# irvingzhang0512/tf_eager_object_detection

Measured on AMD Instinct MI355X. Metric: images/sec, higher is better.
Workload: dtype f32

## Files before the change

tf_eager_object_detection_amd/csrc/nms.hip:

```cpp
#include <stddef.h>
#include <string.h>

#include <algorithm>
#include <mutex>

#include "conv_diag.h"

#define NMS_CHUNK 4096
#define NMS_SEL_MAX (2 * NMS_CHUNK)
#define NMS_WORDS (NMS_CHUNK / 64)
#define SEL_BINS 4096
#define SEL_REPL 8
#define SEL_BLOCK 256
#define SEL_ITEMS 8
#define SEL_TILE (SEL_BLOCK * SEL_ITEMS)
#define PREP_ITEMS 2
#define PREP_TILE (256 * PREP_ITEMS)

typedef unsigned long long u64;

#define SCAN_LDS_BLOCKS 24
#define SCAN_LDS_CAND (SCAN_LDS_BLOCKS * 64)
#define SCAN_LDS_WORDS (SCAN_LDS_BLOCKS * (SCAN_LDS_BLOCKS - 1) / 2 * 64)
#define SCAN_LDS_SLACK_WORDS (8 * 64)
#define SCAN_DYN_LDS ((SCAN_LDS_WORDS + SCAN_LDS_SLACK_WORDS) * 8)
#define SCAN_MAT_OFF(cb, nblk) (64 * ((cb) * ((nblk)-1) - (cb) * ((cb)-1) / 2))

struct NmsState {
  int32_t n_invalid;
  int32_t kept;
  int32_t pos;
  int32_t done;
  int32_t chunk_m;
  int32_t sel_count;
  int32_t reserved0;
  int32_t sel_b1;
  uint32_t sel_below1;
  int32_t sel_b2;
  int32_t sel_overflow;
  uint32_t sel_below;
  int32_t pad[4];
};

#define SEL_COARSE 64
struct NmsHeader {
  NmsState st;
  int32_t n_invalid_acc;
  int32_t pad_acc[15];
  uint32_t hist0[SEL_REPL][SEL_COARSE];
  uint32_t hist1[SEL_REPL][SEL_BINS];
  uint32_t hist2[SEL_BINS];
  uint32_t hist3[256];
};

enum { PREP_NMS = 0, PREP_RP = 1, PREP_FPN = 2, PREP_FRCNN = 3 };

struct PrepParams {
  int n;
  PerImg<const float4*> boxes_in;
  PerImg<const float*> deltas;
  PerImg<const float*> scores;
  PerImg<const float2*> logits;
  Vec4 means, stds;
  float wmax, hmax;
  PerImg<float4*> boxes_out;
  PerImg<uint32_t*> keys;
  PerImg<NmsHeader*> hdr;
  FpnAnchorParams fpn;
};

__global__ void __launch_bounds__(256) k_zero_headers(PerImg<NmsHeader*> hdr_) {
  uint4* d = reinterpret_cast<uint4*>(hdr_.v[blockIdx.y]);
  const int i = blockIdx.x * 256 + threadIdx.x;
  if (i < (int)(sizeof(NmsHeader) / 16)) d[i] = make_uint4(0, 0, 0, 0);
}

template <int MODE>
__device__ __forceinline__ float4 d_prep_box(const PrepParams& p, int img, int e) {
  if (MODE == PREP_NMS) return p.boxes_in.v[img][e];
  float4 a;
  if (MODE == PREP_FPN) {
    a = d_fpn_anchor(p.fpn, e);
  } else if (MODE == PREP_FRCNN) {
    const int ai = e % p.fpn.A, cell = e / p.fpn.A;
    const int x = cell % p.fpn.fw[0], y = cell / p.fpn.fw[0];
    const float sx = (float)(x * p.fpn.stride[0]), sy = (float)(y * p.fpn.stride[0]);
    a = make_float4(p.fpn.wh[ai * 4 + 0] + sx, p.fpn.wh[ai * 4 + 1] + sy, p.fpn.wh[ai * 4 + 2] + sx,
                    p.fpn.wh[ai * 4 + 3] + sy);
  } else {
    a = p.boxes_in.v[img][e];
  }
  const float4 d = reinterpret_cast<const float4*>(p.deltas.v[img])[e];
  const float d0 = d.x * p.stds.v[0] + p.means.v[0];
  const float d1 = d.y * p.stds.v[1] + p.means.v[1];
  const float d2 = d.z * p.stds.v[2] + p.means.v[2];
  const float d3 = d.w * p.stds.v[3] + p.means.v[3];
  float4 b = d_decode_box(a, d0, d1, d2, d3);
  return d_clip_box(b, 0.0f, p.wmax, p.hmax);
}

__device__ __forceinline__ float4 d_candidate_box(const PrepParams& p, int mode, int img, int e) {
  switch (mode) {
    case PREP_NMS: return d_prep_box<PREP_NMS>(p, img, e);
    case PREP_RP: return d_prep_box<PREP_RP>(p, img, e);
    case PREP_FRCNN: return d_prep_box<PREP_FRCNN>(p, img, e);
    default: return d_prep_box<PREP_FPN>(p, img, e);
  }
}

struct PrepItems {
  float sc[PREP_ITEMS];
  float2 lg[PREP_ITEMS];
};

template <int MODE>
__device__ __forceinline__ void d_prep_load(const PrepParams& p, const float* __restrict__ in_scores,
                                            const float2* __restrict__ in_logits, int tile, PrepItems* v) {
#pragma unroll
  for (int it = 0; it < PREP_ITEMS; ++it) {
    const int e = tile * PREP_TILE + it * 256 + threadIdx.x;
    const int ee = e < p.n ? e : 0;
    if (MODE == PREP_FPN) {
      v->lg[it] = in_logits[ee];
    } else if (MODE == PREP_FRCNN) {
      const int loc = ee / p.fpn.A, a = ee - loc * p.fpn.A;
      const float* row = reinterpret_cast<const float*>(in_logits) + (size_t)loc * 2 * p.fpn.A;
      v->lg[it] = make_float2(row[a], row[p.fpn.A + a]);
    } else {
      v->sc[it] = in_scores[ee];
    }
  }
}

__device__ __forceinline__ uint32_t d_row16_sum(uint32_t v) {
  v += (uint32_t)__builtin_amdgcn_update_dpp(0, (int)v, 0xB1, 0xF, 0xF, false);
  v += (uint32_t)__builtin_amdgcn_update_dpp(0, (int)v, 0x4E, 0xF, 0xF, false);
  v += (uint32_t)__builtin_amdgcn_update_dpp(0, (int)v, 0x141, 0xF, 0xF, false);
  v += (uint32_t)__builtin_amdgcn_update_dpp(0, (int)v, 0x140, 0xF, 0xF, false);
  return v;
}

template <int MODE, int T>
__global__ void __launch_bounds__(256) k_rp_prepare(PrepParams p) {
  const int img = blockIdx.y;
  const float* __restrict__ in_scores = p.scores.v[img];
  const float2* __restrict__ in_logits = p.logits.v[img];
  uint32_t* __restrict__ out_keys = p.keys.v[img];
  NmsHeader* hdr = p.hdr.v[img];
  __shared__ __attribute__((aligned(16))) uint32_t h[SEL_BINS];
  uint4* h4 = reinterpret_cast<uint4*>(h);
#pragma unroll
  for (int q = 0; q < SEL_BINS / 4 / 256; ++q) h4[q * 256 + threadIdx.x] = make_uint4(0, 0, 0, 0);
  PrepItems cur;
  d_prep_load<MODE>(p, in_scores, in_logits, blockIdx.x * T, &cur);
  __syncthreads();
  int invalid = 0;
#pragma unroll
  for (int t = 0; t < T; ++t) {
    const int tile = blockIdx.x * T + t;
    PrepItems nxt;
    if (t + 1 < T) d_prep_load<MODE>(p, in_scores, in_logits, tile + 1, &nxt);
#pragma unroll
    for (int it = 0; it < PREP_ITEMS; ++it) {
      const int e = tile * PREP_TILE + it * 256 + threadIdx.x;
      if (e < p.n) {
        float s;
        if (MODE == PREP_FPN || MODE == PREP_FRCNN) s = d_fg_prob(cur.lg[it].x, cur.lg[it].y);
        else s = cur.sc[it];
        const bool valid = s > -3.402823466e+38f;
        const uint32_t k = valid ? ~d_float_asc_key(s) : 0xFFFFFFFFu;
        out_keys[e] = k;
        invalid += valid ? 0 : 1;
        atomicAdd(&h[k >> 20], 1u);
      }
    }
    if (t + 1 < T) cur = nxt;
  }
  __syncthreads();
  const int repl = blockIdx.x % SEL_REPL;
  const int lane = threadIdx.x & 63;
#pragma unroll
  for (int q = 0; q < SEL_BINS / 4 / 256; ++q) {
    const int k4 = q * 256 + threadIdx.x;
    const uint4 c = h4[k4];
    uint32_t s = c.x + c.y + c.z + c.w;
    if (__ballot(s != 0)) {
      const int first = (k4 - lane) * 4;
#pragma unroll
      for (int i = 0; i < 4; ++i) {
        const uint32_t v = h[first + i * 64 + lane];
        if (v) atomicAdd(&hdr->hist1[repl][first + i * 64 + lane], v);
      }
    }
    s = d_row16_sum(s);
    if ((threadIdx.x & 15) == 0 && s) atomicAdd(&hdr->hist0[repl][k4 >> 4], s);
  }
  if (invalid) atomicAdd(&hdr->n_invalid_acc, invalid);
}

template <int REPL>
__device__ __forceinline__ void sel_find(const uint32_t* __restrict__ hist, uint32_t target, uint32_t* result,
                                         int* lds17) {
  uint32_t v[16];
#pragma unroll
  for (int q = 0; q < 16; ++q) v[q] = 0;
#pragma unroll
  for (int r = 0; r < REPL; ++r) {
    const uint4* h4 = reinterpret_cast<const uint4*>(hist + (size_t)r * SEL_BINS) + threadIdx.x * 4;
#pragma unroll
    for (int q = 0; q < 4; ++q) {
      const uint4 t = h4[q];
      v[q * 4 + 0] += t.x; v[q * 4 + 1] += t.y; v[q * 4 + 2] += t.z; v[q * 4 + 3] += t.w;
    }
  }
  uint32_t s = 0;
#pragma unroll
  for (int q = 0; q < 16; ++q) s += v[q];
  int total;
  const uint32_t excl = (uint32_t)block_excl_scan((int)s, lds17, &total);
  if ((uint32_t)total < target) target = (uint32_t)total;
  if (threadIdx.x == 0 && total == 0) { result[0] = SEL_BINS - 1; result[1] = 0; result[2] = 0; }
  if (s > 0 && excl < target && target <= excl + s) {
    uint32_t run = excl;
#pragma unroll
    for (int q = 0; q < 16; ++q) {
      if (run < target && target <= run + v[q]) {
        result[0] = threadIdx.x * 16 + q; result[1] = run; result[2] = v[q];
      }
      run += v[q];
    }
  }
  __syncthreads();
}

__device__ __forceinline__ void sel_find1_coarse(const NmsHeader* hdr, uint32_t target, uint32_t* res) {
  if (threadIdx.x < 64) {
    const int t = threadIdx.x;
    int c = 0;
#pragma unroll
    for (int r = 0; r < SEL_REPL; ++r) c += (int)hdr->hist0[r][t];
    const int inc = wave_incl_scan(c);
    const int total = __shfl(inc, 63);
    if (total == 0) {
      if (t == 0) { res[0] = SEL_BINS - 1; res[1] = 0; }
    } else {
      const int tgt = (int)(target > (uint32_t)total ? (uint32_t)total : target);
      const u64 hitc = __ballot(c > 0 && inc - c < tgt && tgt <= inc);
      const int cb = __builtin_ctzll(hitc);
      const int below_c = __shfl(inc - c, cb);
      int v = 0;
#pragma unroll
      for (int r = 0; r < SEL_REPL; ++r) v += (int)hdr->hist1[r][cb * 64 + t];
      const int inc2 = wave_incl_scan(v);
      const u64 hitf = __ballot(v > 0 && below_c + inc2 - v < tgt && tgt <= below_c + inc2);
      const int fb = __builtin_ctzll(hitf);
      const int below_f = __shfl(inc2 - v, fb);
      if (t == 0) { res[0] = (uint32_t)(cb * 64 + fb); res[1] = (uint32_t)(below_c + below_f); }
    }
  }
  __syncthreads();
}

__global__ void __launch_bounds__(SEL_BLOCK) k_sel_hist2(PerImg<NmsHeader*> hdr_, PerImg<const uint32_t*> keys_, int n,
                                                         uint32_t target) {
  NmsHeader* hdr = hdr_.v[blockIdx.y];
  const uint32_t* __restrict__ keys = keys_.v[blockIdx.y];
  __shared__ uint32_t h[SEL_BINS];
  __shared__ uint32_t res[2];
  uint32_t key[SEL_ITEMS];
#pragma unroll
  for (int it = 0; it < SEL_ITEMS; ++it) {
    const int e = blockIdx.x * SEL_TILE + it * SEL_BLOCK + threadIdx.x;
    key[it] = (e < n) ? keys[e] : 0u;
  }
  sel_find1_coarse(hdr, target, res);
  const uint32_t b1 = res[0];
  if (blockIdx.x == 0 && threadIdx.x == 0) {
    NmsState z;
    memset(&z, 0, sizeof(z));
    z.n_invalid = hdr->n_invalid_acc;
    z.sel_b1 = (int32_t)b1; z.sel_below1 = res[1];
    hdr->st = z;
    hdr->n_invalid_acc = 0;
  }
  bool match = false;
#pragma unroll
  for (int it = 0; it < SEL_ITEMS; ++it) {
    const int e = blockIdx.x * SEL_TILE + it * SEL_BLOCK + threadIdx.x;
    match = match || (e < n && (key[it] >> 20) == b1);
  }
  if (!__syncthreads_or(match ? 1 : 0)) return;
  for (int k = threadIdx.x; k < SEL_BINS; k += SEL_BLOCK) h[k] = 0;
  __syncthreads();
#pragma unroll
  for (int it = 0; it < SEL_ITEMS; ++it) {
    const int e = blockIdx.x * SEL_TILE + it * SEL_BLOCK + threadIdx.x;
    if (e < n && (key[it] >> 20) == b1) atomicAdd(&h[(key[it] >> 8) & 0xFFFu], 1u);
  }
  __syncthreads();
  for (int k = threadIdx.x; k < SEL_BINS; k += SEL_BLOCK) {
    const uint32_t c = h[k];
    if (c) atomicAdd(&hdr->hist2[k], c);
  }
}

__global__ void __launch_bounds__(SEL_BLOCK) k_sel_compact(PerImg<NmsHeader*> hdr_, PerImg<const uint32_t*> keys_, int n,
                                                           uint32_t target, uint32_t limit, PerImg<u64*> cand_) {
  NmsHeader* hdr = hdr_.v[blockIdx.y];
  const uint32_t* __restrict__ keys = keys_.v[blockIdx.y];
  u64* __restrict__ cand = cand_.v[blockIdx.y];
  __shared__ uint32_t res[3];
  __shared__ int lds17[17];
  const uint32_t b1 = (uint32_t)hdr->st.sel_b1;
  const uint32_t below1 = hdr->st.sel_below1;
  {
    static_assert(offsetof(NmsHeader, hist1) == offsetof(NmsHeader, hist0) + sizeof(uint32_t) * SEL_REPL * SEL_COARSE, "layout");
    uint4* z = reinterpret_cast<uint4*>(&hdr->hist0[0][0]);
    for (int i = blockIdx.x * SEL_BLOCK + threadIdx.x; i < SEL_REPL * (SEL_COARSE + SEL_BINS) / 4; i += gridDim.x * SEL_BLOCK)
      z[i] = make_uint4(0, 0, 0, 0);
  }
  uint32_t total_n = (uint32_t)n;
  uint32_t t2 = (target > total_n ? total_n : target) - below1;
  sel_find<1>(hdr->hist2, t2, res, lds17);
  const uint32_t b2 = res[0];
  const bool incl = (below1 + res[1] + res[2]) <= limit;
  if (blockIdx.x == 0 && threadIdx.x == 0) {
    hdr->st.sel_b2 = (int32_t)b2;
    hdr->st.sel_overflow = incl ? 0 : 1;
    hdr->st.sel_below = below1 + res[1];
  }
  __shared__ u64 stage[SEL_TILE];
  __shared__ int s_cnt, s_base;
  if (threadIdx.x == 0) s_cnt = 0;
  uint32_t key[SEL_ITEMS];
#pragma unroll
  for (int it = 0; it < SEL_ITEMS; ++it) {
    const int e = blockIdx.x * SEL_TILE + it * SEL_BLOCK + threadIdx.x;
    key[it] = (e < n) ? keys[e] : 0xFFFFFFFFu;
  }
  __syncthreads();
  const int lane = threadIdx.x & 63;
  const u64 lt_mask = (lane == 0) ? 0ull : (~0ull >> (64 - lane));
#pragma unroll
  for (int it = 0; it < SEL_ITEMS; ++it) {
    const int e = blockIdx.x * SEL_TILE + it * SEL_BLOCK + threadIdx.x;
    const uint32_t k = key[it];
    const uint32_t p1 = k >> 20, p2 = (k >> 8) & 0xFFFu;
    const bool sel = (e < n) && (p1 < b1 || (p1 == b1 && (p2 < b2 || (incl && p2 == b2))));
    const u64 bal = __ballot(sel);
    if (bal) {
      int base = 0;
      if (lane == __builtin_ctzll(bal)) base = atomicAdd(&s_cnt, (int)__popcll(bal));
      base = __shfl(base, __builtin_ctzll(bal));
      if (sel) stage[base + (int)__popcll(bal & lt_mask)] = ((u64)k << 32) | (uint32_t)e;
    }
  }
  __syncthreads();
  const int c = s_cnt;
  if (c == 0) return;
  if (threadIdx.x == 0) s_base = atomicAdd(&hdr->st.sel_count, c);
  __syncthreads();
  const int gb = s_base;
  for (int i = threadIdx.x; i < c; i += SEL_BLOCK)
    if (gb + i < NMS_SEL_MAX) cand[gb + i] = stage[i];
}

__global__ void __launch_bounds__(SEL_BLOCK) k_sel_tie_hist(PerImg<NmsHeader*> hdr_, PerImg<const uint32_t*> keys_, int n,
                                                            PerImg<unsigned short*> bh_) {
  NmsHeader* hdr = hdr_.v[blockIdx.y];
  if (!hdr->st.sel_overflow) return;
  const uint32_t* __restrict__ keys = keys_.v[blockIdx.y];
  unsigned short* __restrict__ bh = bh_.v[blockIdx.y] + (size_t)blockIdx.x * 256;
  __shared__ uint32_t h[256];
  const uint32_t pref = ((uint32_t)hdr->st.sel_b1 << 12) | (uint32_t)hdr->st.sel_b2;
  h[threadIdx.x] = 0;
  __syncthreads();
#pragma unroll
  for (int it = 0; it < SEL_ITEMS; ++it) {
    const int e = blockIdx.x * SEL_TILE + it * SEL_BLOCK + threadIdx.x;
    if (e < n) {
      const uint32_t k = keys[e];
      if ((k >> 8) == pref) atomicAdd(&h[k & 0xFFu], 1u);
    }
  }
  __syncthreads();
  const uint32_t c = h[threadIdx.x];
  bh[threadIdx.x] = (unsigned short)c;
  if (c) atomicAdd(&hdr->hist3[threadIdx.x], c);
}

__global__ void __launch_bounds__(SEL_BLOCK) k_sel_tie_take(PerImg<NmsHeader*> hdr_, PerImg<const uint32_t*> keys_, int n,
                                                            uint32_t limit, PerImg<const unsigned short*> bh_,
                                                            PerImg<u64*> cand_) {
  NmsHeader* hdr = hdr_.v[blockIdx.y];
  if (!hdr->st.sel_overflow) return;
  const uint32_t below = hdr->st.sel_below;
  if (below >= limit) return;
  const uint32_t quota = limit - below;
  const uint32_t* __restrict__ keys = keys_.v[blockIdx.y];
  const unsigned short* __restrict__ bh = bh_.v[blockIdx.y];
  u64* __restrict__ cand = cand_.v[blockIdx.y];
  __shared__ int lds17[17];
  __shared__ uint32_t s_b3, s_q3, s_pre;
  __shared__ int s_wave[4];
  __shared__ u64 stage[SEL_TILE];
  __shared__ int s_cnt, s_base;
  const uint32_t pref = ((uint32_t)hdr->st.sel_b1 << 12) | (uint32_t)hdr->st.sel_b2;
  const uint32_t hv = hdr->hist3[threadIdx.x];
  int total;
  const uint32_t excl = (uint32_t)block_excl_scan((int)hv, lds17, &total);
  if (threadIdx.x == 0) { s_b3 = 256; s_q3 = 0; s_pre = 0; s_cnt = 0; }
  __syncthreads();
  if (hv > 0 && excl < quota && quota <= excl + hv) { s_b3 = threadIdx.x; s_q3 = quota - excl; }
  __syncthreads();
  const uint32_t b3 = s_b3, q3 = s_q3;
  if (b3 < 256) {
    uint32_t mine = 0;
    for (int b = threadIdx.x; b < (int)blockIdx.x; b += SEL_BLOCK) mine += bh[(size_t)b * 256 + b3];
    int tot2;
    block_excl_scan((int)mine, lds17, &tot2);
    if (threadIdx.x == 0) s_pre = (uint32_t)tot2;
  }
  __syncthreads();
  uint32_t run = s_pre;
  const int lane = threadIdx.x & 63, wv = threadIdx.x >> 6;
  const u64 lt_mask = (lane == 0) ? 0ull : (~0ull >> (64 - lane));
  for (int it = 0; it < SEL_ITEMS; ++it) {
    const int e = blockIdx.x * SEL_TILE + it * SEL_BLOCK + threadIdx.x;
    const uint32_t k = (e < n) ? keys[e] : 0xFFFFFFFFu;
    const bool inbin = (e < n) && (k >> 8) == pref;
    const uint32_t v = k & 0xFFu;
    const bool tie = inbin && v == b3;
    const u64 tb = __ballot(tie);
    if (lane == 0) s_wave[wv] = (int)__popcll(tb);
    __syncthreads();
    uint32_t before = run;
    for (int q = 0; q < wv; ++q) before += (uint32_t)s_wave[q];
    const uint32_t my_rank = before + (uint32_t)__popcll(tb & lt_mask);
    const uint32_t all4 = (uint32_t)(s_wave[0] + s_wave[1] + s_wave[2] + s_wave[3]);
    const bool sel = inbin && (v < b3 || (tie && my_rank < q3));
    const u64 bal = __ballot(sel);
    if (bal) {
      int base = 0;
      if (lane == __builtin_ctzll(bal)) base = atomicAdd(&s_cnt, (int)__popcll(bal));
      base = __shfl(base, __builtin_ctzll(bal));
      if (sel) stage[base + (int)__popcll(bal & lt_mask)] = ((u64)k << 32) | (uint32_t)e;
    }
    run += all4;
    __syncthreads();
  }
  const int c = s_cnt;
  if (c == 0) return;
  if (threadIdx.x == 0) s_base = atomicAdd(&hdr->st.sel_count, c);
  __syncthreads();
  const int gb = s_base;
  for (int i = threadIdx.x; i < c; i += SEL_BLOCK)
    if (gb + i < NMS_SEL_MAX) cand[gb + i] = stage[i];
}

#define RANK_THREADS 1024
__global__ void __launch_bounds__(RANK_THREADS) k_sel_rank(PerImg<NmsHeader*> hdr_, int n, int cap0, PerImg<const u64*> cand_,
                                                          PrepParams prep, int mode, PerImg<uint32_t*> sel_idx_,
                                                          PerImg<float4*> sboxes_, PerImg<float4*> sorig_) {
  NmsHeader* hdr = hdr_.v[blockIdx.y];
  const u64* __restrict__ cand = cand_.v[blockIdx.y];
  uint32_t* __restrict__ sel_idx = sel_idx_.v[blockIdx.y];
  float4* __restrict__ sboxes = sboxes_.v[blockIdx.y];
  float4* __restrict__ sorig = sorig_.v[blockIdx.y];
  __shared__ u64 all[NMS_CHUNK];
  __shared__ int part[16][64];
  NmsState* st = &hdr->st;
  const int cnt = min(st->sel_count, NMS_SEL_MAX);
  if (blockIdx.x == 0 && threadIdx.x == 0) st->chunk_m = min(min(cnt, cap0), n - st->n_invalid);
  if (blockIdx.x == 0) {
    uint4* z = reinterpret_cast<uint4*>(hdr->hist2);
    for (int i = threadIdx.x; i < SEL_BINS / 4; i += RANK_THREADS) z[i] = make_uint4(0, 0, 0, 0);
    if (threadIdx.x < 256) hdr->hist3[threadIdx.x] = 0;
  }
  if (blockIdx.x * 64 >= cnt) return;
  const int lane = threadIdx.x & 63, w = threadIdx.x >> 6;
  const int i = blockIdx.x * 64 + lane;
  const u64 mine = (i < cnt) ? cand[i] : ~0ull;
  float4 bx = make_float4(0.0f, 0.0f, 0.0f, 0.0f);
  if (w == 0 && i < cnt) bx = d_candidate_box(prep, mode, blockIdx.y, (int)(uint32_t)mine);
  int c = 0;
  for (int t0 = 0; t0 < cnt; t0 += NMS_CHUNK) {
    const int tc = min(NMS_CHUNK, cnt - t0);
    __syncthreads();
    for (int k = threadIdx.x; k < tc; k += RANK_THREADS) all[k] = cand[t0 + k];
    __syncthreads();
    const int per = (tc + 15) >> 4;
    const int lo = w * per, hi = min(tc, lo + per);
    for (int j = lo; j < hi; ++j) c += (all[j] < mine) ? 1 : 0;
  }
  part[w][lane] = c;
  __syncthreads();
  if (w == 0 && i < cnt) {
    int r = 0;
#pragma unroll
    for (int k = 0; k < 16; ++k) r += part[k][lane];
    const uint32_t idx = (uint32_t)mine;
    sel_idx[r] = idx;
    if (r < cap0) {
      sboxes[r] = d_norm_box(bx);
      sorig[r] = bx;
    }
  }
}

__global__ void __launch_bounds__(256) k_nms_gather(PerImg<NmsState*> st_, int n, int cap, int from_sel,
                                                    PrepParams prep, int mode, PerImg<const uint32_t*> sorted_idx_,
                                                    PerImg<float4*> sboxes_, PerImg<float4*> sorig_) {
  NmsState* st = st_.v[blockIdx.y];
  const uint32_t* __restrict__ sorted_idx = sorted_idx_.v[blockIdx.y];
  float4* __restrict__ sboxes = sboxes_.v[blockIdx.y];
  float4* __restrict__ sorig = sorig_.v[blockIdx.y];
  const int pos = st->pos, nv = n - st->n_invalid;
  const int lim = from_sel ? min(nv, min(st->sel_count, NMS_SEL_MAX)) : nv;
  const int m = st->done ? 0 : max(0, min(cap, lim - pos));
  const int i = blockIdx.x * 256 + threadIdx.x;
  if (i == 0) st->chunk_m = m;
  if (i < m) {
    const float4 bx = d_candidate_box(prep, mode, blockIdx.y, (int)sorted_idx[pos + i]);
    sboxes[i] = d_norm_box(bx);
    sorig[i] = bx;
  }
}

__global__ void __launch_bounds__(256) k_nms_cross(PerImg<const NmsState*> st_, PerImg<const float4*> sboxes_,
                                                   PerImg<const float4*> kept_boxes_, float thr,
                                                   PerImg<u64*> removed_init_) {
  const NmsState* st = st_.v[blockIdx.y];
  const float4* __restrict__ sboxes = sboxes_.v[blockIdx.y];
  const float4* __restrict__ kept_boxes = kept_boxes_.v[blockIdx.y];
  u64* __restrict__ removed_init = removed_init_.v[blockIdx.y];
  __shared__ float4 kb[256];
  __shared__ float ka[256];
  const int m = st->chunk_m, nk = st->kept;
  if (blockIdx.x * 256 >= m) return;
  const int j = blockIdx.x * 256 + threadIdx.x;
  const float4 b = (j < m) ? sboxes[j] : make_float4(0, 0, 0, 0);
  const float area = d_box_area(b);
  bool sup = false;
  for (int k0 = 0; k0 < nk; k0 += 256) {
    __syncthreads();
    if (k0 + threadIdx.x < nk) {
      float4 t = kept_boxes[k0 + threadIdx.x];
      kb[threadIdx.x] = t;
      ka[threadIdx.x] = d_box_area(t);
    }
    __syncthreads();
    const int lim = min(256, nk - k0);
    for (int k = 0; k < lim; ++k) sup = sup || d_iou_gt(b, area, kb[k], ka[k], thr);
  }
  u64 bal = __ballot(sup && j < m);
  if ((threadIdx.x & 63) == 0) removed_init[j >> 6] = bal;
}

__global__ void __launch_bounds__(256) k_nms_mask(PerImg<const NmsState*> st_, PerImg<const float4*> sboxes_, float thr,
                                                  PerImg<u64*> Lt_, PerImg<u64*> diag_, int packed) {
  const NmsState* st = st_.v[blockIdx.y];
  const float4* __restrict__ sboxes = sboxes_.v[blockIdx.y];
  u64* __restrict__ Lt = Lt_.v[blockIdx.y];
  u64* __restrict__ diag_up = diag_.v[blockIdx.y];
  const int t = blockIdx.x;
  int rb = (int)((sqrtf(8.0f * (float)t + 1.0f) - 1.0f) * 0.5f);
  while ((rb + 1) * (rb + 2) / 2 <= t) ++rb;
  while (rb * (rb + 1) / 2 > t) --rb;
  const int cb = t - rb * (rb + 1) / 2;
  const int m = st->chunk_m;
  if (rb * 64 >= m) return;
  __shared__ float4 cbox[64];
  __shared__ float carea[64];
  __shared__ uint32_t part[4][64];
  const int lane = threadIdx.x & 63, w = threadIdx.x >> 6;
  if (threadIdx.x < 64) {
    const int col = cb * 64 + lane;
    const float4 c = (col < m) ? sboxes[col] : make_float4(0, 0, 0, 0);
    cbox[lane] = c;
    carea[lane] = d_box_area(c);
  }
  __syncthreads();
  const int row = rb * 64 + lane;
  const float4 r = (row < m) ? sboxes[row] : make_float4(0, 0, 0, 0);
  const float ra = d_box_area(r);
  uint32_t bits = 0;
#pragma unroll
  for (int j = 0; j < 16; ++j) {
    const int jj = w * 16 + j;
    const bool s = d_iou_gt(r, ra, cbox[jj], carea[jj], thr);
    bits |= s ? (1u << j) : 0u;
  }
  part[w][lane] = bits;
  __syncthreads();
  if (w == 0 && row < m) {
    const u64 word = (u64)part[0][lane] | ((u64)part[1][lane] << 16) | ((u64)part[2][lane] << 32) |
                     ((u64)part[3][lane] << 48);
    if (cb == rb) {
      const u64 later = (lane == 63) ? 0ull : (~0ull << (lane + 1));
      diag_up[row] = word & later;
    } else {
      if (packed) Lt[SCAN_MAT_OFF(cb, (m + 63) >> 6) + row - (cb + 1) * 64] = word;
      else Lt[(size_t)cb * NMS_CHUNK + row] = word;
    }
  }
}

struct AssignOut {
  float4* rois;
  int32_t* level;
  int64_t* perm;
  int32_t* counts;
  int32_t* order;
  int min_level, max_level;
};

#define SCAN_THREADS 512
#define SCAN_WAVES (SCAN_THREADS / 64)
#define SCAN_Q 8
#define SCAN_RING 4
#define SCAN_STAGE_ITEMS ((SCAN_LDS_WORDS / 2 + SCAN_THREADS - 1) / SCAN_THREADS)

__device__ __forceinline__ u64 rfl64(u64 v) {
  uint32_t lo = __builtin_amdgcn_readfirstlane((uint32_t)v);
  uint32_t hi = __builtin_amdgcn_readfirstlane((uint32_t)(v >> 32));
  return ((u64)hi << 32) | lo;
}

__device__ __forceinline__ u64 scan_resolve_block(u64 alive, u64 d, int room, int lane, u64 lt_lane, int* npop_out) {
  const uint32_t dlo = (uint32_t)d, dhi = (uint32_t)(d >> 32);
  for (;;) {
    const bool is_s = ((alive >> lane) & 1ull) && ((d & alive) != 0ull);
    const u64 supp = __ballot(is_s);
    if (supp == 0) break;
    const int i = __builtin_ctzll(supp);
    const uint32_t rlo = __builtin_amdgcn_readlane(dlo, i);
    const uint32_t rhi = __builtin_amdgcn_readlane(dhi, i);
    alive &= ~(((u64)rhi << 32) | rlo);
  }
  const int npop = (int)__popcll(alive);
  u64 kept = alive;
  if (npop > room) kept = __ballot(((alive >> lane) & 1ull) && (int)__popcll(alive & lt_lane) < room);
  *npop_out = min(npop, room);
  return kept;
}

__device__ __forceinline__ u64 scan_wait_block(const int* nkeptw, const u64* keepw, int b, int* nk) {
  int v;
  u64 kbv;
  for (;;) {
    v = __hip_atomic_load(&nkeptw[b], __ATOMIC_RELAXED, __HIP_MEMORY_SCOPE_WORKGROUP);
    asm volatile("" ::: "memory");
    kbv = __hip_atomic_load(&keepw[b], __ATOMIC_RELAXED, __HIP_MEMORY_SCOPE_WORKGROUP);
    if (v >= 0) break;
    __builtin_amdgcn_s_sleep(1);
  }
  *nk = __builtin_amdgcn_readfirstlane(v);
  return rfl64(kbv);
}

__device__ __forceinline__ void scan_publish(int* nkeptw, u64* keepw, int b, u64 kept, int nk, int lane) {
  if (lane == 0) __hip_atomic_store(&keepw[b], kept, __ATOMIC_RELAXED, __HIP_MEMORY_SCOPE_WORKGROUP);
  asm volatile("s_waitcnt lgkmcnt(0)" ::: "memory");
  if (lane == 0) __hip_atomic_store(&nkeptw[b], nk, __ATOMIC_RELAXED, __HIP_MEMORY_SCOPE_WORKGROUP);
}

struct ScanParams {
  PerImg<NmsState*> st;
  PerImg<const u64*> Lt, diag_up, removed_init;
  PerImg<const float4*> sboxes, sorig;
  PerImg<const uint32_t*> sorted_idx;
  PerImg<int32_t*> out_idx;
  PerImg<float4*> out_boxes, kept_boxes;
  PerImg<int32_t*> out_count, out_done;
// ... 981 lines not shown
```

tf_eager_object_detection_amd/csrc/odet_internal.h:

```cpp
#ifndef ODET_INTERNAL_H_
#define ODET_INTERNAL_H_

#include <hip/hip_runtime.h>
#include <stdint.h>
#include <stdio.h>

#include <mutex>

#include "../../include/odet.h"

#define ODET_WAVE 64

int odet_set_error(int code, const char* fmt, ...);

#define ODET_REQUIRE(cond, ...)                                   \
  do {                                                            \
    if (!(cond)) return odet_set_error(ODET_E_INVALID, __VA_ARGS__); \
  } while (0)

#define ODET_HIP(call)                                                                      \
  do {                                                                                      \
    hipError_t e_ = (call);                                                                 \
    if (e_ != hipSuccess)                                                                   \
      return odet_set_error(ODET_E_HIP, "%s failed: %s (%s:%d)", #call, hipGetErrorString(e_), \
                            __FILE__, __LINE__);                                            \
  } while (0)

#define ODET_LAUNCH_CHECK() ODET_HIP(hipGetLastError())

struct OdetPerDeviceOnce {
  static constexpr int MAXDEV = 64;
  std::once_flag once[MAXDEV];
  hipError_t rc[MAXDEV];
  template <typename F>
  hipError_t run(F fn) {
    int dev = 0;
    const hipError_t eg = hipGetDevice(&dev);
    if (eg != hipSuccess) return eg;
    if (dev < 0 || dev >= MAXDEV) return hipErrorInvalidDevice;
    std::call_once(once[dev], [&] { rc[dev] = fn(); });
    return rc[dev];
  }
};

static inline size_t odet_align_up(size_t v, size_t a) { return (v + a - 1) / a * a; }

struct OdetArena {
  char* base;
  size_t size;
  size_t off;
  template <typename T>
  T* take(size_t count) {
    size_t o = odet_align_up(off, 256);
    size_t end = o + count * sizeof(T);
    if (end > size) return nullptr;
    off = end;
    return reinterpret_cast<T*>(base + o);
  }
};

#ifdef __HIPCC__
enum { TG_STREAM_ANCHOR_FG = 0, TG_STREAM_ANCHOR_BG = 1, TG_STREAM_ROI_FG = 2, TG_STREAM_ROI_BG = 3, TG_STREAM_ROI_REPLACE = 4,
       TG_STREAM_IMAGE_FLIP = 5, TG_STREAM_DROPOUT_FC1 = 6, TG_STREAM_DROPOUT_FC2 = 7 };

__host__ __device__ __forceinline__ void odet_philox4(uint32_t c0, uint32_t c1, uint32_t c2, uint32_t c3, uint32_t k0,
                                                      uint32_t k1, uint32_t* w) {
#pragma unroll
  for (int r = 0; r < 10; ++r) {
    const unsigned long long p0 = (unsigned long long)0xD2511F53u * c0, p1 = (unsigned long long)0xCD9E8D57u * c2;
    const uint32_t hi0 = (uint32_t)(p0 >> 32), lo0 = (uint32_t)p0;
    const uint32_t hi1 = (uint32_t)(p1 >> 32), lo1 = (uint32_t)p1;
    c0 = hi1 ^ c1 ^ k0; c1 = lo1; c2 = hi0 ^ c3 ^ k1; c3 = lo0;
    k0 += 0x9E3779B9u; k1 += 0xBB67AE85u;
  }
  w[0] = c0; w[1] = c1; w[2] = c2; w[3] = c3;
}

__host__ __device__ __forceinline__ void odet_philox2(uint32_t c0, uint32_t c1, uint32_t c2, uint32_t c3, uint32_t k0,
                                                      uint32_t k1, uint32_t* w0, uint32_t* w1) {
  uint32_t w[4];
  odet_philox4(c0, c1, c2, c3, k0, k1, w);
  *w0 = w[0]; *w1 = w[1];
}

__device__ __forceinline__ float d_exp32(float x) { return (float)exp((double)x); }
__device__ __forceinline__ float d_log32(float x) { return (float)log((double)x); }

__device__ __forceinline__ float4 d_norm_box(float4 b) {
  return make_float4(fminf(b.x, b.z), fminf(b.y, b.w), fmaxf(b.x, b.z), fmaxf(b.y, b.w));
}
__device__ __forceinline__ float d_box_area(float4 nb) { return (nb.z - nb.x) * (nb.w - nb.y); }
__device__ __forceinline__ bool d_iou_gt(float4 a, float area_a, float4 b, float area_b, float thr) {
  if (area_a <= 0.0f || area_b <= 0.0f) return false;
  float i0 = fmaxf(a.x, b.x), i1 = fmaxf(a.y, b.y);
  float i2 = fminf(a.z, b.z), i3 = fminf(a.w, b.w);
  float inter = fmaxf(i2 - i0, 0.0f) * fmaxf(i3 - i1, 0.0f);
  float iou = inter / (area_a + area_b - inter);
  return iou > thr;
}

__device__ __forceinline__ float4 d_decode_box(float4 a, float d0, float d1, float d2, float d3) {
  float width = a.z - a.x + 1.0f;
  float height = a.w - a.y + 1.0f;
  float cx = a.x + 0.5f * width;
  float cy = a.y + 0.5f * height;
  cx = cx + d0 * width;
  cy = cy + d1 * height;
  width = width * d_exp32(d2);
  height = height * d_exp32(d3);
  float x1 = cx - 0.5f * width;
  float y1 = cy - 0.5f * height;
  return make_float4(x1, y1, x1 + width, y1 + height);
}

__device__ __forceinline__ float4 d_clip_box(float4 b, float minv, float wmax, float hmax) {
  return make_float4(fmaxf(fminf(b.x, wmax), minv), fmaxf(fminf(b.y, hmax), minv),
                     fmaxf(fminf(b.z, wmax), minv), fmaxf(fminf(b.w, hmax), minv));
}

__device__ __forceinline__ float d_pair_iou(float4 p, float4 q) {
  float a1 = (p.w - p.y + 1.0f) * (p.z - p.x + 1.0f);
  float a2 = (q.w - q.y + 1.0f) * (q.z - q.x + 1.0f);
  float ih = fmaxf(0.0f, fminf(p.w, q.w) - fmaxf(p.y, q.y) + 1.0f);
  float iw = fmaxf(0.0f, fminf(p.z, q.z) - fmaxf(p.x, q.x) + 1.0f);
  float inter = ih * iw;
  float uni = a1 + a2 - inter;
  return (inter == 0.0f) ? 0.0f : inter / uni;
}

__device__ __forceinline__ float4 d_encode_box(float4 b, float4 g, const float* means, const float* stds) {
  float width = b.z - b.x + 1.0f, height = b.w - b.y + 1.0f;
  float cx = b.x + 0.5f * width, cy = b.y + 0.5f * height;
  float gw = g.z - g.x + 1.0f, gh = g.w - g.y + 1.0f;
  float gcx = g.x + 0.5f * gw, gcy = g.y + 0.5f * gh;
  float dx = (gcx - cx) / width;
  float dy = (gcy - cy) / height;
  float dw = d_log32(gw / width);
  float dh = d_log32(gh / height);
  return make_float4((dx - means[0]) / stds[0], (dy - means[1]) / stds[1],
                     (dw - means[2]) / stds[2], (dh - means[3]) / stds[3]);
}

__device__ __forceinline__ uint32_t d_float_asc_key(float f) {
  uint32_t u = __float_as_uint(f);
  return (u & 0x80000000u) ? ~u : (u | 0x80000000u);
}
#endif


struct Vec4 { float v[4]; };

#define ODET_MAX_BATCH 8
template <typename T>
struct PerImg {
  T v[ODET_MAX_BATCH];
};

struct FpnAnchorParams {
  int num_levels;
  int A;
  int fw[ODET_MAX_LEVELS];
  int stride[ODET_MAX_LEVELS];
  int start[ODET_MAX_LEVELS + 1];
  float wh[ODET_MAX_LEVELS * ODET_MAX_ANCHORS_PER_CELL * 2];
};

#ifdef __HIPCC__
__device__ __forceinline__ float4 d_fpn_anchor(const FpnAnchorParams& p, int i) {
  int l = 0;
#pragma unroll
  for (int k = 1; k < ODET_MAX_LEVELS; ++k)
    if (k < p.num_levels && i >= p.start[k]) l = k;
  int j = i - p.start[l];
  int a = j % p.A;
  int cell = j / p.A;
  int x = cell % p.fw[l], y = cell / p.fw[l];
  float fs = (float)p.stride[l];
  float cx = (float)x * fs, cy = (float)y * fs;
  float hw = 0.5f * p.wh[(l * p.A + a) * 2 + 0];
  float hh = 0.5f * p.wh[(l * p.A + a) * 2 + 1];
  return make_float4(cx - hw, cy - hh, cx + hw, cy + hh);
// ... 267 lines not shown
```

tf_eager_object_detection_amd/csrc/postops.hip:

```cpp
#include <mutex>

#include "odet_internal.h"

#define PO_THREADS 1024
#define PO_ROUND 128

typedef unsigned long long u64;

static int next_pow2_(int v) {
  int p = 1;
  while (p < v) p <<= 1;
  return p;
}

struct PostOpsParams {
  PerImg<const float*> scores_t;
  PerImg<const float*> deltas_t;
  PerImg<const float4*> rois_t;
  PerImg<const int32_t*> count_dev_t;
  int R, Ccls, P2, K;
  float means[4], stds[4];
  float wmax, hmax, min_edge, score_thr, nms_thr;
  float roi_div;
  PerImg<int32_t*> cls_count_t;
// ... 106 lines not shown
        ++o;
      }
    }
    if (tid == 0) *p.out_count = kept_total;
    return;
  }
  int nlt = 0, neq = 0;
  for (int q = 0; q < per; ++q) {
    const int slot = lo + q;
    if (slot < nslots) {
      const uint32_t k = key[slot];
      if (k != 0xFFFFFFFFu) { nlt += (k < T || M == total) ? 1 : 0; neq += (k == T && M < total) ? 1 : 0; }
    }
  }
  int tot_eq, tot_lt;
  int eq_before = block_excl_scan(neq, lds17, &tot_eq);
  int sel_before = block_excl_scan(nlt + max(0, min(neq, (int)min((u64)take_ties, (u64)0x7FFFFFFF) - eq_before)), lds17, &tot_lt);
  {
    int o = sel_before, e = eq_before;
    for (int q = 0; q < per; ++q) {
      const int slot = lo + q;
      if (slot < nslots) {
        const uint32_t k = key[slot];
        bool sel = false;
        if (k != 0xFFFFFFFFu) {
          if (k < T || M == total) sel = true;
          else if (k == T) { sel = (uint32_t)e < take_ties; ++e; }
        }
        if (sel && o < M) { sel_key[o] = k; sel_slot[o] = (uint32_t)slot; ++o; }
      }
    }
  }
  __syncthreads();
  for (int i = tid; i < M; i += PO_THREADS) {
    const uint32_t ki = sel_key[i], si = sel_slot[i];
    int rank = 0;
    for (int j = 0; j < M; ++j) {
      const uint32_t kj = sel_key[j], sj = sel_slot[j];
      rank += (kj < ki || (kj == ki && sj < si)) ? 1 : 0;
    }
    const float4 b = p.cls_boxes[si];
    const float sc = p.cls_scores[si];
    const int lab = (int)(si / (uint32_t)p.K) + 1;
    p.out_boxes[rank] = b;
    p.out_scores[rank] = sc;
    p.out_labels[rank] = lab;
    if (p.out_record) {
      float* r = p.out_record + (size_t)rank * 6;
      r[0] = b.x; r[1] = b.y; r[2] = b.z; r[3] = b.w; r[4] = sc; r[5] = (float)lab;
    }
  }
  if (p.out_record) {
    for (int i = M + tid; i < p.max_per_image; i += PO_THREADS) {
      float* r = p.out_record + (size_t)i * 6;
      r[0] = 0.0f; r[1] = 0.0f; r[2] = 0.0f; r[3] = 0.0f; r[4] = -1.0f; r[5] = 0.0f;
    }
  }
  if (tid == 0) {
    *p.out_count = M;
    if (p.out_record) p.out_record[(size_t)p.max_per_image * 6] = (float)M;
  }
}

__global__ void __launch_bounds__(PO_THREADS) k_postops(PostOpsParams p) {
  extern __shared__ __align__(16) unsigned char smem[];
  const int img = blockIdx.y;
  const float* __restrict__ in_scores = p.scores_t.v[img];
  const float* __restrict__ in_deltas = p.deltas_t.v[img];
  const float4* __restrict__ in_rois = p.rois_t.v[img];
  const int32_t* __restrict__ in_count = p.count_dev_t.v[img];
  int32_t* __restrict__ cls_count = p.cls_count_t.v[img];
  float4* __restrict__ cls_boxes = p.cls_boxes_t.v[img];
  float* __restrict__ cls_scores = p.cls_scores_t.v[img];
  const int nkeys = p.P2 > 2048 ? p.P2 : 2048;
  u64* keys = reinterpret_cast<u64*>(smem);
  float4* lbox = reinterpret_cast<float4*>(keys + nkeys);
  float4* sbox = lbox + p.R;
  float4* kbox = sbox + PO_ROUND;
  u64* mask = reinterpret_cast<u64*>(kbox + p.K);
  float* sarea = reinterpret_cast<float*>(mask + PO_ROUND * 2);
  float* karea = sarea + PO_ROUND;
  uint32_t* crossf = reinterpret_cast<uint32_t*>(karea + p.K);
  __shared__ int s_nvalid, s_nk, s_last;

  const int c = blockIdx.x + 1;
  const int tid = threadIdx.x, lane = tid & 63, w = tid >> 6;
  if (tid == 0) { s_nvalid = 0; s_nk = 0; s_last = 0; }

  const int Rdev = in_count ? *in_count : p.R;
  u64 mykey = ~0ull;
  for (int r = tid; r < p.P2; r += PO_THREADS) {
    u64 key = ~0ull;
    if (r < p.R) {
      const float s = in_scores[(size_t)r * p.Ccls + c];
      const float4 t = *reinterpret_cast<const float4*>(in_deltas + ((size_t)r * p.Ccls + c) * 4);
      float4 roi = in_rois[r];
      if (r < min(Rdev, p.R) && s > p.score_thr) {
        const float d0 = t.x * p.stds[0] + p.means[0];
        const float d1 = t.y * p.stds[1] + p.means[1];
        const float d2 = t.z * p.stds[2] + p.means[2];
        const float d3 = t.w * p.stds[3] + p.means[3];
        if (p.roi_div != 1.0f) {
          roi.x = roi.x / p.roi_div; roi.y = roi.y / p.roi_div; roi.z = roi.z / p.roi_div; roi.w = roi.w / p.roi_div;
        }
        float4 b = d_decode_box(roi, d0, d1, d2, d3);
        b = d_clip_box(b, 0.0f, p.wmax, p.hmax);
        const float e0 = b.z - b.x + 1.0f, e1 = b.w - b.y + 1.0f;
        if (e1 >= p.min_edge && e0 >= p.min_edge) {
          lbox[r] = b;
          key = ((u64)(~d_float_asc_key(s)) << 32) | (unsigned)r;
        }
      }
    }
    if (p.P2 > 1024) keys[r] = key; else mykey = key;
  }
  __syncthreads();
  {
    const u64 bal = __ballot(p.P2 <= 1024 && mykey != ~0ull);
    if (lane == 0 && bal) atomicAdd(&s_nvalid, (int)__popcll(bal));
  }
  __syncthreads();

  if (p.P2 <= 1024) {
    mykey = bitonic_sort_1024_reg(mykey, keys);
    __syncthreads();
    keys[tid] = mykey;
    __syncthreads();
  } else {
    bitonic_sort_u64(keys, p.P2, PO_THREADS);
    if (tid == 0) {
      int lo = 0, hi = p.P2;
      while (lo < hi) { int mid = (lo + hi) >> 1; if (keys[mid] != ~0ull) lo = mid + 1; else hi = mid; }
      s_nvalid = lo;
    }
    __syncthreads();
  }
  const int nvalid = s_nvalid;
  const int K = p.K;

  const u64 lt_lane = (lane == 0) ? 0ull : (~0ull >> (64 - lane));
  for (int t0 = 0; t0 < nvalid; t0 += PO_ROUND) {
    const int nk0 = s_nk;
    if (nk0 >= K) break;
    const int mround = min(PO_ROUND, nvalid - t0);
    if (tid < PO_ROUND) {
      float4 nb = make_float4(0, 0, 0, 0);
      if (tid < mround) nb = d_norm_box(lbox[(int)(keys[t0 + tid] & 0xFFFFFFFFull)]);
      sbox[tid] = nb;
      sarea[tid] = d_box_area(nb);
      crossf[tid] = 0;
    }
    __syncthreads();
    {
      const int row = tid & (PO_ROUND - 1), cs = tid >> 7;
      const float4 rb = sbox[row];
      const float ra = sarea[row];
      uint32_t bits = 0;
#pragma unroll
      for (int j = 0; j < 16; ++j) {
        const int col = cs * 16 + j;
        const bool s = (col < row) && d_iou_gt(rb, ra, sbox[col], sarea[col], p.nms_thr);
        bits |= s ? (1u << j) : 0u;
      }
      reinterpret_cast<unsigned short*>(mask)[row * 8 + cs] = (unsigned short)bits;
      bool sup = false;
      for (int k = cs; k < nk0; k += 8) sup = sup || d_iou_gt(rb, ra, kbox[k], karea[k], p.nms_thr);
      if (sup) atomicOr(&crossf[row], 1u);
    }
    __syncthreads();
    if (w == 0) {
      int nk = nk0;
      u64 kept0 = 0;
#pragma unroll
      for (int blk = 0; blk < 2; ++blk) {
        const int row = blk * 64 + lane;
        const u64 m0 = mask[row * 2 + 0], m1 = mask[row * 2 + 1];
        bool dead = (row >= mround) || (crossf[row] != 0);
        if (blk == 1) dead = dead || ((m0 & kept0) != 0ull);
        const u64 mm = (blk == 0) ? m0 : m1;
        u64 alive = __ballot(!dead);
        u64 kept = 0;
        while (alive != 0 && nk < K) {
          const int i = __builtin_ctzll(alive);
          kept |= 1ull << i;
          ++nk;
          alive &= ~(1ull << i);
          alive &= ~__ballot((mm >> i) & 1ull);
        }
        if (blk == 0) kept0 = kept;
        if ((kept >> lane) & 1ull) {
          const int slot = nk0 + (blk == 1 ? (int)__popcll(kept0) : 0) + (int)__popcll(kept & lt_lane);
          const u64 kk = keys[t0 + row];
          const float4 ob = lbox[(int)(kk & 0xFFFFFFFFull)];
          kbox[slot] = sbox[row];
          karea[slot] = sarea[row];
          cls_boxes[(size_t)blockIdx.x * K + slot] = ob;
          cls_scores[(size_t)blockIdx.x * K + slot] = key_to_score((uint32_t)(kk >> 32));
        }
      }
      if (lane == 0) s_nk = nk;
    }
    __syncthreads();
  }
  if (tid == 0) cls_count[blockIdx.x] = s_nk;

  asm volatile("s_waitcnt vmcnt(0)" ::: "memory");
  __syncthreads();
  if (tid == 0) {
    __builtin_amdgcn_fence(__ATOMIC_RELEASE, "agent");
    asm volatile("s_waitcnt vmcnt(0)" ::: "memory");
    const uint32_t t = atomicInc(p.ticket_t.v[img], (uint32_t)(p.ncls1 - 1));
    s_last = (t == (uint32_t)(p.ncls1 - 1)) ? 1 : 0;
  }
  __syncthreads();
  if (!s_last) return;
  if (tid == 0) __builtin_amdgcn_fence(__ATOMIC_ACQUIRE, "agent");
  asm volatile("s_waitcnt vmcnt(0)" ::: "memory");
  __syncthreads();
  MergeView mv;
  mv.cls_count = cls_count; mv.cls_boxes = cls_boxes; mv.cls_scores = cls_scores;
  mv.ncls1 = p.ncls1; mv.K = p.K; mv.max_per_image = p.max_per_image; mv.mode = p.mode;
  mv.out_boxes = p.out_boxes_t.v[img]; mv.out_labels = p.out_labels_t.v[img]; mv.out_scores = p.out_scores_t.v[img];
  mv.out_count = p.out_count_t.v[img]; mv.out_record = p.out_record_t.v[img];
  postops_merge(mv, smem);
}

extern "C" size_t odet_post_ops_workspace_bytes(int num_classes, int max_per_class) {
  size_t n1 = (size_t)(num_classes > 1 ? num_classes - 1 : 1);
  size_t k = (size_t)(max_per_class > 0 ? max_per_class : 1);
  return odet_align_up(n1 * 4, 256) + odet_align_up(n1 * k * 16, 256) + odet_align_up(n1 * k * 4, 256) + 1024;
}

int odet_post_ops_batch(const PostOpsImageIO* io, int B, int R, int Ccls, int num_classes, PostOpsExtra ex,
                        const float* means, const float* stds, int max_per_class, int max_per_image,
                        float nms_iou_threshold, float score_threshold, float min_edge, hipStream_t st, int ws_clean) {
  ODET_REQUIRE(io && B >= 1 && B <= ODET_MAX_BATCH, "odet_post_ops: bad batch");
  ODET_REQUIRE(R >= 0 && Ccls > 0 && num_classes >= 1 && num_classes <= Ccls, "odet_post_ops: bad sizes");
  ODET_REQUIRE(max_per_class >= 0 && max_per_image >= 0, "odet_post_ops: negative cap");
  for (int i = 0; i < B; ++i) ODET_REQUIRE(io[i].out_count, "odet_post_ops: null out_count");
  if (R == 0 || num_classes == 1 || max_per_class == 0 || (max_per_image == 0 && ex.mode == 0)) {
    for (int i = 0; i < B; ++i) {
      ODET_HIP(hipMemsetAsync(io[i].out_count, 0, sizeof(int32_t), st));
      if (io[i].out_record && max_per_image > 0) {
        int rc = odet_pack_detections(io[i].out_boxes, io[i].out_labels, io[i].out_scores, io[i].out_count, 0,
                                      max_per_image, io[i].out_record, (odet_stream_t)st);
        if (rc != ODET_OK) return rc;
      }
    }
    return ODET_OK;
// ... 146 lines not shown
```

Measured before the change: 30030.

## Use division-free IoU test with exact fallback and coarse hist2 selection

```diff
diff --git a/tf_eager_object_detection_amd/csrc/nms.hip b/tf_eager_object_detection_amd/csrc/nms.hip
--- a/tf_eager_object_detection_amd/csrc/nms.hip
+++ b/tf_eager_object_detection_amd/csrc/nms.hip
@@ -51,6 +51,7 @@
   uint32_t hist1[SEL_REPL][SEL_BINS];
   uint32_t hist2[SEL_BINS];
   uint32_t hist3[256];
+  uint32_t hist2c[SEL_COARSE];
 };
 
 enum { PREP_NMS = 0, PREP_RP = 1, PREP_FPN = 2, PREP_FRCNN = 3 };
@@ -199,50 +200,17 @@
 }
 
 template <int REPL>
-__device__ __forceinline__ void sel_find(const uint32_t* __restrict__ hist, uint32_t target, uint32_t* result,
-                                         int* lds17) {
-  uint32_t v[16];
-#pragma unroll
-  for (int q = 0; q < 16; ++q) v[q] = 0;
-#pragma unroll
-  for (int r = 0; r < REPL; ++r) {
-    const uint4* h4 = reinterpret_cast<const uint4*>(hist + (size_t)r * SEL_BINS) + threadIdx.x * 4;
-#pragma unroll
-    for (int q = 0; q < 4; ++q) {
-      const uint4 t = h4[q];
-      v[q * 4 + 0] += t.x; v[q * 4 + 1] += t.y; v[q * 4 + 2] += t.z; v[q * 4 + 3] += t.w;
-    }
-  }
-  uint32_t s = 0;
-#pragma unroll
-  for (int q = 0; q < 16; ++q) s += v[q];
-  int total;
-  const uint32_t excl = (uint32_t)block_excl_scan((int)s, lds17, &total);
-  if ((uint32_t)total < target) target = (uint32_t)total;
-  if (threadIdx.x == 0 && total == 0) { result[0] = SEL_BINS - 1; result[1] = 0; result[2] = 0; }
-  if (s > 0 && excl < target && target <= excl + s) {
-    uint32_t run = excl;
-#pragma unroll
-    for (int q = 0; q < 16; ++q) {
-      if (run < target && target <= run + v[q]) {
-        result[0] = threadIdx.x * 16 + q; result[1] = run; result[2] = v[q];
-      }
-      run += v[q];
-    }
-  }
-  __syncthreads();
-}
-
-__device__ __forceinline__ void sel_find1_coarse(const NmsHeader* hdr, uint32_t target, uint32_t* res) {
+__device__ __forceinline__ void sel_find_coarse(const uint32_t* __restrict__ coarse, const uint32_t* __restrict__ fine,
+                                                uint32_t target, uint32_t* res) {
   if (threadIdx.x < 64) {
     const int t = threadIdx.x;
     int c = 0;
 #pragma unroll
-    for (int r = 0; r < SEL_REPL; ++r) c += (int)hdr->hist0[r][t];
+    for (int r = 0; r < REPL; ++r) c += (int)coarse[r * SEL_COARSE + t];
     const int inc = wave_incl_scan(c);
     const int total = __shfl(inc, 63);
     if (total == 0) {
-      if (t == 0) { res[0] = SEL_BINS - 1; res[1] = 0; }
+      if (t == 0) { res[0] = SEL_BINS - 1; res[1] = 0; if (REPL == 1) res[2] = 0; }
     } else {
       const int tgt = (int)(target > (uint32_t)total ? (uint32_t)total : target);
       const u64 hitc = __ballot(c > 0 && inc - c < tgt && tgt <= inc);
@@ -250,12 +218,16 @@
       const int below_c = __shfl(inc - c, cb);
       int v = 0;
 #pragma unroll
-      for (int r = 0; r < SEL_REPL; ++r) v += (int)hdr->hist1[r][cb * 64 + t];
+      for (int r = 0; r < REPL; ++r) v += (int)fine[r * SEL_BINS + cb * 64 + t];
       const int inc2 = wave_incl_scan(v);
       const u64 hitf = __ballot(v > 0 && below_c + inc2 - v < tgt && tgt <= below_c + inc2);
       const int fb = __builtin_ctzll(hitf);
       const int below_f = __shfl(inc2 - v, fb);
-      if (t == 0) { res[0] = (uint32_t)(cb * 64 + fb); res[1] = (uint32_t)(below_c + below_f); }
+      const int count_f = __shfl(v, fb);
+      if (t == 0) {
+        res[0] = (uint32_t)(cb * 64 + fb); res[1] = (uint32_t)(below_c + below_f);
+        if (REPL == 1) res[2] = (uint32_t)count_f;
+      }
     }
   }
   __syncthreads();
@@ -265,7 +237,7 @@
                                                          uint32_t target) {
   NmsHeader* hdr = hdr_.v[blockIdx.y];
   const uint32_t* __restrict__ keys = keys_.v[blockIdx.y];
-  __shared__ uint32_t h[SEL_BINS];
+  __shared__ __attribute__((aligned(16))) uint32_t h[SEL_BINS];
   __shared__ uint32_t res[2];
   uint32_t key[SEL_ITEMS];
 #pragma unroll
@@ -273,7 +245,7 @@
     const int e = blockIdx.x * SEL_TILE + it * SEL_BLOCK + threadIdx.x;
     key[it] = (e < n) ? keys[e] : 0u;
   }
-  sel_find1_coarse(hdr, target, res);
+  sel_find_coarse<SEL_REPL>(&hdr->hist0[0][0], &hdr->hist1[0][0], target, res);
   const uint32_t b1 = res[0];
   if (blockIdx.x == 0 && threadIdx.x == 0) {
     NmsState z;
@@ -298,9 +270,29 @@
     if (e < n && (key[it] >> 20) == b1) atomicAdd(&h[(key[it] >> 8) & 0xFFFu], 1u);
   }
   __syncthreads();
-  for (int k = threadIdx.x; k < SEL_BINS; k += SEL_BLOCK) {
-    const uint32_t c = h[k];
-    if (c) atomicAdd(&hdr->hist2[k], c);
+  __shared__ uint32_t csum[SEL_COARSE];
+  const uint4* h4 = reinterpret_cast<const uint4*>(h);
+  const int lane = threadIdx.x & 63;
+#pragma unroll
+  for (int q = 0; q < SEL_BINS / 4 / SEL_BLOCK; ++q) {
+    const int k4 = q * SEL_BLOCK + threadIdx.x;
+    const uint4 c = h4[k4];
+    uint32_t s = c.x + c.y + c.z + c.w;
+    if (__ballot(s != 0)) {
+      const int first = (k4 - lane) * 4;
+#pragma unroll
+      for (int i = 0; i < 4; ++i) {
+        const uint32_t v = h[first + i * 64 + lane];
+        if (v) atomicAdd(&hdr->hist2[first + i * 64 + lane], v);
+      }
+    }
+    s = d_row16_sum(s);
+    if ((threadIdx.x & 15) == 0) csum[k4 >> 4] = s;
+  }
+  __syncthreads();
+  if (threadIdx.x < SEL_COARSE) {
+    const uint32_t v = csum[threadIdx.x];
+    if (v) atomicAdd(&hdr->hist2c[threadIdx.x], v);
   }
 }
 
@@ -310,7 +302,6 @@
   const uint32_t* __restrict__ keys = keys_.v[blockIdx.y];
   u64* __restrict__ cand = cand_.v[blockIdx.y];
   __shared__ uint32_t res[3];
-  __shared__ int lds17[17];
   const uint32_t b1 = (uint32_t)hdr->st.sel_b1;
   const uint32_t below1 = hdr->st.sel_below1;
   {
@@ -321,7 +312,7 @@
   }
   uint32_t total_n = (uint32_t)n;
   uint32_t t2 = (target > total_n ? total_n : target) - below1;
-  sel_find<1>(hdr->hist2, t2, res, lds17);
+  sel_find_coarse<1>(hdr->hist2c, hdr->hist2, t2, res);
   const uint32_t b2 = res[0];
   const bool incl = (below1 + res[1] + res[2]) <= limit;
   if (blockIdx.x == 0 && threadIdx.x == 0) {
@@ -476,6 +467,7 @@
     uint4* z = reinterpret_cast<uint4*>(hdr->hist2);
     for (int i = threadIdx.x; i < SEL_BINS / 4; i += RANK_THREADS) z[i] = make_uint4(0, 0, 0, 0);
     if (threadIdx.x < 256) hdr->hist3[threadIdx.x] = 0;
+    if (threadIdx.x < SEL_COARSE) hdr->hist2c[threadIdx.x] = 0;
   }
   if (blockIdx.x * 64 >= cnt) return;
   const int lane = threadIdx.x & 63, w = threadIdx.x >> 6;
@@ -536,22 +528,44 @@
   u64* __restrict__ removed_init = removed_init_.v[blockIdx.y];
   __shared__ float4 kb[256];
   __shared__ float ka[256];
+  __shared__ uint32_t kposm[8];
   const int m = st->chunk_m, nk = st->kept;
   if (blockIdx.x * 256 >= m) return;
   const int j = blockIdx.x * 256 + threadIdx.x;
   const float4 b = (j < m) ? sboxes[j] : make_float4(0, 0, 0, 0);
   const float area = d_box_area(b);
+  const bool apos = area > 0.0f;
   bool sup = false;
+  uint32_t kpos = 0;
   for (int k0 = 0; k0 < nk; k0 += 256) {
     __syncthreads();
-    if (k0 + threadIdx.x < nk) {
-      float4 t = kept_boxes[k0 + threadIdx.x];
-      kb[threadIdx.x] = t;
-      ka[threadIdx.x] = d_box_area(t);
+    {
+      float ta = 0.0f;
+      if (k0 + threadIdx.x < nk) {
+        float4 t = kept_boxes[k0 + threadIdx.x];
+        kb[threadIdx.x] = t;
+        ta = d_box_area(t);
+        ka[threadIdx.x] = ta;
+      }
+      const u64 pm = __ballot(ta > 0.0f);
+      if ((threadIdx.x & 63) == 0) { kposm[threadIdx.x >> 5] = (uint32_t)pm; kposm[(threadIdx.x >> 5) + 1] = (uint32_t)(pm >> 32); }
     }
     __syncthreads();
     const int lim = min(256, nk - k0);
-    for (int k = 0; k < lim; ++k) sup = sup || d_iou_gt(b, area, kb[k], ka[k], thr);
+    bool hit = false, unsure = false;
+    for (int k = 0; k < lim; ++k) {
+      if ((k & 31) == 0) kpos = (uint32_t)__builtin_amdgcn_readfirstlane((int)kposm[k >> 5]);
+      hit |= d_iou_gt_try(apos && ((kpos >> (k & 31)) & 1u), b, area, kb[k], ka[k], thr, &unsure);
+    }
+    if (__ballot(unsure)) {
+      hit = false;
+#pragma unroll 1
+      for (int k = 0; k < lim; ++k) {
+        kpos = (uint32_t)__builtin_amdgcn_readfirstlane((int)kposm[k >> 5]);
+        hit |= d_iou_gt_div(apos && ((kpos >> (k & 31)) & 1u), b, area, kb[k], ka[k], thr);
+      }
+    }
+    sup |= hit;
   }
   u64 bal = __ballot(sup && j < m);
   if ((threadIdx.x & 63) == 0) removed_init[j >> 6] = bal;
@@ -573,23 +587,39 @@
   __shared__ float4 cbox[64];
   __shared__ float carea[64];
   __shared__ uint32_t part[4][64];
+  __shared__ uint32_t cposm[4];
   const int lane = threadIdx.x & 63, w = threadIdx.x >> 6;
   if (threadIdx.x < 64) {
     const int col = cb * 64 + lane;
     const float4 c = (col < m) ? sboxes[col] : make_float4(0, 0, 0, 0);
+    const float ca = d_box_area(c);
     cbox[lane] = c;
-    carea[lane] = d_box_area(c);
+    carea[lane] = ca;
+    const u64 pm = __ballot(ca > 0.0f);
+    if (lane < 4) cposm[lane] = (uint32_t)(pm >> (16 * lane)) & 0xFFFFu;
   }
   __syncthreads();
   const int row = rb * 64 + lane;
   const float4 r = (row < m) ? sboxes[row] : make_float4(0, 0, 0, 0);
   const float ra = d_box_area(r);
+  const bool rpos = ra > 0.0f;
+  const uint32_t cpos = (uint32_t)__builtin_amdgcn_readfirstlane((int)cposm[w]);
   uint32_t bits = 0;
-#pragma unroll
+  bool unsure = false;
+#pragma unroll 4
   for (int j = 0; j < 16; ++j) {
     const int jj = w * 16 + j;
-    const bool s = d_iou_gt(r, ra, cbox[jj], carea[jj], thr);
+    const bool s = d_iou_gt_try(rpos && ((cpos >> j) & 1u), r, ra, cbox[jj], carea[jj], thr, &unsure);
     bits |= s ? (1u << j) : 0u;
+  }
+  if (__ballot(unsure)) {
+    bits = 0;
+#pragma unroll 1
+    for (int j = 0; j < 16; ++j) {
+      const int jj = w * 16 + j;
+      const bool s = d_iou_gt_div(rpos && ((cpos >> j) & 1u), r, ra, cbox[jj], carea[jj], thr);
+      bits |= s ? (1u << j) : 0u;
+    }
   }
   part[w][lane] = bits;
   __syncthreads();
diff --git a/tf_eager_object_detection_amd/csrc/odet_internal.h b/tf_eager_object_detection_amd/csrc/odet_internal.h
--- a/tf_eager_object_detection_amd/csrc/odet_internal.h
+++ b/tf_eager_object_detection_amd/csrc/odet_internal.h
@@ -90,13 +90,36 @@
   return make_float4(fminf(b.x, b.z), fminf(b.y, b.w), fmaxf(b.x, b.z), fmaxf(b.y, b.w));
 }
 __device__ __forceinline__ float d_box_area(float4 nb) { return (nb.z - nb.x) * (nb.w - nb.y); }
+__device__ __forceinline__ float d_max_nb(float x, float y) {
+  float r;
+  asm("v_max_f32 %0, %1, %2" : "=v"(r) : "v"(x), "v"(y));
+  return r;
+}
+__device__ __forceinline__ float d_min_nb(float x, float y) {
+  float r;
+  asm("v_min_f32 %0, %1, %2" : "=v"(r) : "v"(x), "v"(y));
+  return r;
+}
+__device__ __forceinline__ float d_iou_inter(float4 a, float4 b) {
+  float i0 = d_max_nb(a.x, b.x), i1 = d_max_nb(a.y, b.y);
+  float i2 = d_min_nb(a.z, b.z), i3 = d_min_nb(a.w, b.w);
+  return fmaxf(i2 - i0, 0.0f) * fmaxf(i3 - i1, 0.0f);
+}
+__device__ __forceinline__ bool d_iou_gt_div(bool need, float4 a, float area_a, float4 b, float area_b, float thr) {
+  const float inter = d_iou_inter(a, b);
+  const float iou = inter / (area_a + area_b - inter);
+  return need && iou > thr;
+}
+__device__ __forceinline__ bool d_iou_gt_try(bool need, float4 a, float area_a, float4 b, float area_b, float thr, bool* unsure) {
+  const float inter = d_iou_inter(a, b);
+  const float u = area_a + area_b - inter;
+  const float t = thr * u;
+  const bool sure = thr >= 0x1p-126f && thr <= 0x1.fffffep+127f && __builtin_amdgcn_classf(t, 0x100) && fabsf(inter - t) > 0x1p-21f * t;
+  *unsure = *unsure || (need && !sure);
+  return need && inter > t;
+}
 __device__ __forceinline__ bool d_iou_gt(float4 a, float area_a, float4 b, float area_b, float thr) {
-  if (area_a <= 0.0f || area_b <= 0.0f) return false;
-  float i0 = fmaxf(a.x, b.x), i1 = fmaxf(a.y, b.y);
-  float i2 = fminf(a.z, b.z), i3 = fminf(a.w, b.w);
-  float inter = fmaxf(i2 - i0, 0.0f) * fmaxf(i3 - i1, 0.0f);
-  float iou = inter / (area_a + area_b - inter);
-  return iou > thr;
+  return d_iou_gt_div(area_a > 0.0f && area_b > 0.0f, a, area_a, b, area_b, thr);
 }
 
 __device__ __forceinline__ float4 d_decode_box(float4 a, float d0, float d1, float d2, float d3) {
diff --git a/tf_eager_object_detection_amd/csrc/postops.hip b/tf_eager_object_detection_amd/csrc/postops.hip
--- a/tf_eager_object_detection_amd/csrc/postops.hip
+++ b/tf_eager_object_detection_amd/csrc/postops.hip
@@ -212,6 +212,7 @@
   float* karea = sarea + PO_ROUND;
   uint32_t* crossf = reinterpret_cast<uint32_t*>(karea + p.K);
   __shared__ int s_nvalid, s_nk, s_last;
+  __shared__ uint32_t s_cpos[PO_ROUND / 16];
 
   const int c = blockIdx.x + 1;
   const int tid = threadIdx.x, lane = tid & 63, w = tid >> 6;
@@ -276,25 +277,46 @@
     if (tid < PO_ROUND) {
       float4 nb = make_float4(0, 0, 0, 0);
       if (tid < mround) nb = d_norm_box(lbox[(int)(keys[t0 + tid] & 0xFFFFFFFFull)]);
+      const float na = d_box_area(nb);
       sbox[tid] = nb;
-      sarea[tid] = d_box_area(nb);
+      sarea[tid] = na;
       crossf[tid] = 0;
+      const u64 pm = __ballot(na > 0.0f);
+      if (lane < 4) s_cpos[w * 4 + lane] = (uint32_t)(pm >> (16 * lane)) & 0xFFFFu;
     }
     __syncthreads();
     {
       const int row = tid & (PO_ROUND - 1), cs = tid >> 7;
       const float4 rb = sbox[row];
       const float ra = sarea[row];
+      const bool rpos = ra > 0.0f;
+      const uint32_t cpos = (uint32_t)__builtin_amdgcn_readfirstlane((int)s_cpos[cs]);
       uint32_t bits = 0;
-#pragma unroll
+      bool unsure = false;
+#pragma unroll 4
       for (int j = 0; j < 16; ++j) {
         const int col = cs * 16 + j;
-        const bool s = (col < row) && d_iou_gt(rb, ra, sbox[col], sarea[col], p.nms_thr);
+        const bool s = d_iou_gt_try(rpos && ((cpos >> j) & 1u) && (col < row), rb, ra, sbox[col], sarea[col], p.nms_thr, &unsure);
         bits |= s ? (1u << j) : 0u;
+      }
+      if (__ballot(unsure)) {
+        bits = 0;
+#pragma unroll 1
+        for (int j = 0; j < 16; ++j) {
+          const int col = cs * 16 + j;
+          const bool s = d_iou_gt_div(rpos && ((cpos >> j) & 1u) && (col < row), rb, ra, sbox[col], sarea[col], p.nms_thr);
+          bits |= s ? (1u << j) : 0u;
+        }
       }
       reinterpret_cast<unsigned short*>(mask)[row * 8 + cs] = (unsigned short)bits;
       bool sup = false;
-      for (int k = cs; k < nk0; k += 8) sup = sup || d_iou_gt(rb, ra, kbox[k], karea[k], p.nms_thr);
+      unsure = false;
+      for (int k = cs; k < nk0; k += 8) sup |= d_iou_gt_try(rpos && karea[k] > 0.0f, rb, ra, kbox[k], karea[k], p.nms_thr, &unsure);
+      if (__ballot(unsure)) {
+        sup = false;
+#pragma unroll 1
+        for (int k = cs; k < nk0; k += 8) sup |= d_iou_gt_div(rpos && karea[k] > 0.0f, rb, ra, kbox[k], karea[k], p.nms_thr);
+      }
       if (sup) atomicOr(&crossf[row], 1u);
     }
     __syncthreads();
```

After: 29940. No clear change (-0.3%).
